# yupbank/tensorframes

Hardware: AMD Instinct MI355X
Metric: rows/sec map_blocks MatMul on 10M-row DF at 1/2/4/8 MI355X (higher is better)
Workload: dtype fp32; 1 GPU; model=map_blocks relu(matmul(x[?,512], W[512,512])) float32, global_batch=10000000, seq_len=512, parallelism=dp1, partitions=4, rows=10000000

## Files before the change

### csrc/runtime/executor.cpp

```cpp
#include "executor.h"

#include <optional>
#include "device_pool.h"


#include <ATen/hip/HIPContext.h>
#include <c10/hip/HIPCachingAllocator.h>
#include <c10/hip/HIPGuard.h>
#include <hip/hip_runtime.h>
#include <rocprofiler-sdk-roctx/roctx.h>

#include <algorithm>
#include <array>
#include <atomic>
#include <chrono>
#include <condition_variable>
#include <deque>
#include <thread>
#include <unistd.h>
#include <cstdlib>
#include <set>
#include <unordered_map>
#include <sstream>

// ... 1271 lines not shown
  p.arenas[di] = std::move(ar);
}

void Program::refresh_consts(Plan& p, int di, void* stream) {
  p.stale.erase(di);
  auto& m = p.dev_consts[di];
  if (m.empty()) return;
  auto drop = [&]() {
    m.clear();
    p.arenas.erase(di);
    p.cap_reset = true;
  };
  if (di < 0) {
    m.clear();
    return;
  }
  auto ait = p.arenas.find(di);
  if (ait == p.arenas.end()) return drop();
  Plan::Arena& ar = ait->second;
  std::set<int> in_arena;
  for (auto& it : ar.items) in_arena.insert(std::get<0>(it));
  for (auto& kv : m)
    if (!in_arena.count(kv.first) && kv.second.numel() > 0) return drop();
  at::Tensor host = at::empty({ar.dev.numel()}, at::TensorOptions().dtype(at::kByte).pinned_memory(true));
  auto* hp = static_cast<uint8_t*>(host.data_ptr());
  for (auto& it : ar.items) {
    const TensorRef& r = std::get<1>(it);
    const auto& v = p.infos[r.node][r.index].value;
    if (!v) return drop();
    at::Tensor c = v->contiguous();
    if (static_cast<size_t>(c.nbytes()) != std::get<3>(it)) return drop();
    std::memcpy(hp + std::get<2>(it), c.data_ptr(), c.nbytes());
  }
  hipStream_t s = static_cast<hipStream_t>(stream);
  for (void* us : p.used_streams[di])
    if (us && us != stream) (void)hipStreamSynchronize(static_cast<hipStream_t>(us));
  {
    c10::hip::HIPStreamGuard sg(c10::hip::getStreamFromExternal(s, static_cast<c10::DeviceIndex>(di)));
    ar.dev.copy_(host, true);
  }
  void*& ev = const_events_[{di, stream}];
  if (!ev) {
    hipEvent_t e;
    TFA_CHECK(hipEventCreateWithFlags(&e, hipEventDisableTiming) == hipSuccess, "hipEventCreate failed");
    ev = e;
  }
  (void)hipEventRecord(static_cast<hipEvent_t>(ev), s);
}

std::shared_ptr<Program> Program::rebind(const std::map<std::string, at::Tensor>& values) {
  static const bool timing = [] {
    const char* e = std::getenv("TFA_PLAN_TIMING");
    return e && std::string(e) == "3";
  }();
  const auto t0 = std::chrono::steady_clock::now();
  auto g = g_->with_values(values);
  const auto t1 = std::chrono::steady_clock::now();
  auto p = std::make_shared<Program>(std::move(g), fetch_names_, feed_names_);
  const auto t2 = std::chrono::steady_clock::now();
  p->adopt(*this);
  if (timing) {
    const auto t3 = std::chrono::steady_clock::now();
    auto us = [](auto a, auto b) { return std::chrono::duration<double, std::micro>(b - a).count(); };
    std::fprintf(stderr, "[tfa rebind] with_values %.1fus program %.1fus adopt %.1fus\n", us(t0, t1), us(t1, t2),
                 us(t2, t3));
  }
  return p;
}

bool Program::adopt(Program& old) {
  if (&old == this) return false;
  if (g_->structure_key() != old.g_->structure_key() || g_->nodes().size() != old.g_->nodes().size())
    return false;
  if (fetch_names_ != old.fetch_names_ || feed_names_ != old.feed_names_ || order_ != old.order_) return false;
  if (!host_op_error_.empty() || !old.host_op_error_.empty()) return false;
  std::scoped_lock lk(mu_, old.mu_, const_mu_, old.const_mu_);
  if (!plans_.empty()) return false;
  for (auto& kv : old.plans_) {
    if (!kv.second->synth_consts.empty()) return false;
    if (kv.second.use_count() != 1) return false;
  }
  std::vector<std::pair<std::shared_ptr<Plan>, Graph::Infos>> fresh;
  const std::vector<char>& prm = g_->parameter_consts();
  std::vector<char> redo(g_->nodes().size(), 0);
  for (int n : order_) {
    char t = prm[n];
    for (auto& r : g_->node(n).inputs) t = t || redo[r.node];
    redo[n] = t;
  }
  for (auto& kv : old.plans_) {
    Plan& p = *kv.second;
    Graph::Infos ni = p.infos.size() == g_->nodes().size() ? g_->infer_update(order_, p.infos, redo, true)
                                                           : g_->infer(order_, p.feed_infos, true);
    for (auto& cs : p.const_slots) {
      const TensorRef& r = cs.second;
      const TensorInfo& a = p.infos[r.node][r.index];
      const TensorInfo& b = ni[r.node][r.index];
      if (a.dtype != b.dtype || a.shape.dims != b.shape.dims || !b.value || !a.value ||
          a.value->sizes() != b.value->sizes())
        return false;
    }
    fresh.emplace_back(kv.second, std::move(ni));
  }
  for (auto& [pp, ni] : fresh) {
    Plan& p = *pp;
    for (auto& cs : p.const_slots) {
      const TensorRef& r = cs.second;
      p.infos[r.node][r.index].value = ni[r.node][r.index].value;
    }
    for (size_t n = 0; n < redo.size() && n < p.infos.size(); ++n)
      if (redo[n])
        for (size_t k = 0; k < p.infos[n].size() && k < ni[n].size(); ++k) p.infos[n][k].value = ni[n][k].value;
    for (auto& kv : p.dev_consts)
      if (!kv.second.empty()) p.stale.insert(kv.first);
  }
  plans_ = std::move(old.plans_);
  old.plans_.clear();
  old.graph_consts_.clear();
  for (auto& kv : old.const_events_) {
    void*& ev = const_events_[kv.first];
    if (ev) (void)hipEventDestroy(static_cast<hipEvent_t>(ev));
    ev = kv.second;
  }
  old.const_events_.clear();
  stats_.plans_adopted += static_cast<int64_t>(plans_.size());
  return true;
}

void Program::wait_consts(const at::Device& dev, void* stream) {
  std::lock_guard<std::mutex> lk(const_mu_);
  if (const_events_.empty()) return;
  const int di = dev.index();
  hipStream_t s = static_cast<hipStream_t>(stream);
  for (auto it = const_events_.begin(); it != const_events_.end();) {
    hipEvent_t e = static_cast<hipEvent_t>(it->second);
    if (it->first.first != di) {
      ++it;
      continue;
    }
    if (hipEventQuery(e) == hipSuccess) {
      (void)hipEventDestroy(e);
      it = const_events_.erase(it);
      continue;
    }
    if (it->first.second != stream && !dev_stream_capturing(s)) (void)hipStreamWaitEvent(s, e, 0);
    ++it;
  }
}

Program::~Program() {
  {
    std::lock_guard<std::mutex> lk(pipe_mu_);
    drop_pipe(false);
  }
  for (auto& kv : const_events_) (void)hipEventDestroy(static_cast<hipEvent_t>(kv.second));
}

std::vector<at::Tensor> Program::execute(Plan& p, const std::vector<at::Tensor>& inputs, void* stream) {
  const auto t_exec = std::chrono::steady_clock::now();
  auto epi_steps = [](const Step& st, const std::vector<at::Tensor>& slots) {
    std::vector<EpiStep> ep;
    for (const auto& e : st.epi) {
      EpiStep x;
      x.code = e.code;
      x.kind = e.kind;
      x.act = e.act;
      x.s = e.s;
      if (e.slot >= 0) x.t = slots[e.slot].contiguous();
      ep.push_back(std::move(x));
    }
    return ep;
  };
  const OpRegistry& reg = OpRegistry::get();
  at::Device dev = inputs.empty() ? at::Device(at::kCPU) : inputs[0].device();
  bool gpu = dev.is_cuda();
  for (auto& t : inputs)
    TFA_CHECK(t.device() == dev, "all inputs must live on the same device");
  std::vector<at::Tensor> slots(p.nslots);
  for (size_t i = 0; i < inputs.size(); ++i) slots[p.feed_slots[i]] = inputs[i].contiguous();
  if (!p.stale.empty()) {
    std::lock_guard<std::mutex> lk(const_mu_);
    const int di = gpu ? dev.index() : -1;
    if (p.stale.count(di)) refresh_consts(p, di, stream);
  }
  for (auto& cs : p.const_slots) slots[cs.first] = device_const(p, cs.first, dev, stream);
  if (gpu) {
    wait_consts(dev, stream);
    std::lock_guard<std::mutex> lk(const_mu_);
    p.last_stream[dev.index()] = stream;
    if (!dev_stream_capturing(static_cast<hipStream_t>(stream))) p.used_streams[dev.index()].insert(stream);
  }
  for (auto& sc : p.synth_consts) {
    std::lock_guard<std::mutex> lk(const_mu_);
    auto& m = p.dev_consts[dev.is_cuda() ? dev.index() : -1];
    auto it = m.find(sc.first);
    if (it == m.end()) it = m.emplace(sc.first, dev.is_cuda() ? sc.second.to(dev) : sc.second).first;
    slots[sc.first] = it->second;
  }
  const bool timing = gpu && g_step_timing.load(std::memory_order_relaxed) &&
                      !dev_stream_capturing(static_cast<hipStream_t>(stream));
  for (auto& st : p.steps) {
    const Node& nd = g_->node(st.node);
    ExecCtx c{nd, {}, {}, &st.out_info, &st.in_info, gpu, stream};
    for (int s : st.in_slots) c.in.push_back(slots[s]);
    c.out.resize(st.out_info.size());
    StepRec rec;
    if (timing) {
      TFA_CHECK(hipEventCreate(&rec.a) == hipSuccess, "hipEventCreate failed");
      TFA_CHECK(hipEventCreate(&rec.b) == hipSuccess, "hipEventCreate failed");
      TFA_CHECK(hipEventRecord(rec.a, static_cast<hipStream_t>(stream)) == hipSuccess, "hipEventRecord failed");
    }
    {
      std::unique_ptr<RangeGuard> rg;
      if (gpu) rg = std::make_unique<RangeGuard>(nd.op + ":" + nd.name);
      try {
        if (st.kind == Step::FUSED) {
          TFA_CHECK(gpu, "internal: fused step in a host plan");
          Plan::Fused& fe = *p.fused_regions[st.fused];
          const int di = dev.index();
          jit::Kernel kern;
          {
            std::lock_guard<std::mutex> lk(fe.mu);
            auto kit = fe.kernels.find(di);
            if (kit == fe.kernels.end()) {
              hipStreamCaptureStatus cs = hipStreamCaptureStatusNone;
              (void)hipStreamIsCapturing(static_cast<hipStream_t>(stream), &cs);
              TFA_CHECK(cs == hipStreamCaptureStatusNone, "fused kernel not loaded before graph capture");
              kit = fe.kernels.emplace(di, jit::get(fe.region.source, fe.region.entry)).first;
            }
            kern = kit->second;
          }
          std::vector<void*> outs;
          for (size_t k = 0; k < st.out_slots.size(); ++k) {
            c.out[k] = c.alloc_out(static_cast<int>(k));
            outs.push_back(c.out[k].data_ptr());
          }
          std::vector<const void*> ptrs;
          for (size_t k = 0; k < c.in.size(); ++k) {
            if (!c.in[k].is_contiguous()) c.in[k] = materialize(c, c.in[k]);
            ptrs.push_back(c.in[k].data_ptr());
          }
          std::vector<int64_t> w = fused_args(fe.region, ptrs, outs);
          TFA_CHECK(fe.region.grid >= 1 && fe.region.grid < (int64_t(1) << 31), "fused kernel: grid out of range");
          jit::launch(kern, static_cast<unsigned>(fe.region.grid), fe.region.block, w.data(),
                      w.size() * sizeof(int64_t), static_cast<hipStream_t>(stream));
        } else if (st.kind == Step::OP && gpu && !st.preplaced.empty()) {
          if (st.alias_slot >= 0) {
            at::Tensor& whole = slots[st.alias_slot];
            if (!whole.defined())
              whole = dev_empty(dims_or_throw(st.alias_info->shape, "concat output"), at::kFloat, dev,
                                static_cast<hipStream_t>(stream));
            slots[st.out_slots[0]] = whole.narrow(whole.dim() - 1, st.alias_offset, st.out_info[0].shape.dims.back());
          }
          at::Tensor& out = slots[st.out_slots[0]];
          TFA_CHECK(out.defined(), "internal: concat output not allocated by its producers");
          int64_t off = 0;
          const int64_t ax = out.dim() - 1;
          for (size_t v = 0; v < st.preplaced.size(); ++v) {
            const int64_t len = c.in[v].size(ax);
            if (!st.preplaced[v] && len > 0) gpu_copy(c.in[v], out.narrow(ax, off, len), stream_of(c));
            off += len;
          }
          c.out[0] = out;
        } else if (st.kind == Step::OP && gpu && (st.bias_slot >= 0 || st.act || st.alias_slot >= 0) &&
                   (nd.op == "AvgPool" || nd.op == "MaxPool")) {
          at::Tensor out;
          if (st.alias_slot >= 0) {
            at::Tensor& whole = slots[st.alias_slot];
            if (!whole.defined())
              whole = dev_empty(dims_or_throw(st.alias_info->shape, "concat output"), at::kFloat, dev,
                                static_cast<hipStream_t>(stream));
            out = whole.narrow(whole.dim() - 1, st.alias_offset, st.out_info[0].shape.dims.back());
          } else {
            out = c.alloc_out(0);
          }
          at::Tensor bias;
          if (st.bias_slot >= 0) bias = slots[st.bias_slot].contiguous();
          run_pool_fused(c, nd.op == "MaxPool", c.in[0], st.bias_slot >= 0 ? &bias : nullptr, st.act, out);
          c.out[0] = out;
        } else if (st.kind == Step::OP) {
          reg.find(nd.op)->compute(c);
        } else if (!st.sibs.empty()) {
          TFA_CHECK(gpu, "internal: sibling-fused conv in a host plan");
          std::vector<at::Tensor> outs;
          for (size_t k = 0; k < st.sibs.size(); ++k) {
            const Step::Sib& sb = st.sibs[k];
            if (sb.alias_slot >= 0) {
              at::Tensor& whole = slots[sb.alias_slot];
              if (!whole.defined())
                whole = dev_empty(dims_or_throw(sb.alias_info->shape, "concat output"), at::kFloat, dev,
                                  static_cast<hipStream_t>(stream));
              outs.push_back(whole.narrow(whole.dim() - 1, sb.alias_offset, sb.oc));
            } else {
              outs.push_back(c.alloc_out(static_cast<int>(k)));
            }
          }
          at::Tensor bias;
          if (st.bias_slot >= 0) bias = slots[st.bias_slot];
          std::vector<int> acts;
          for (const auto& sb : st.sibs) acts.push_back(sb.act);
          run_conv2d_siblings(c, c.in[0], c.in[1], st.bias_slot >= 0 ? &bias : nullptr, st.act, outs, acts,
                              st.wino_slot >= 0 ? &slots[st.wino_slot] : nullptr);
          for (size_t k = 0; k < outs.size(); ++k) c.out[k] = outs[k];
        } else if (gpu && st.alias_slot >= 0) {
          at::Tensor& whole = slots[st.alias_slot];
          if (!whole.defined())
// ... 544 lines not shown
    std::unique_lock<std::mutex> lk(mu);
    cv.wait(lk, [&] { return posted; });
    for (auto& j : jobs) {
      if (!j) continue;
      try {
        j->wait();
      } catch (const std::exception& e) {
        if (error.empty()) error = e.what();
      }
      j.reset();
    }
    TFA_CHECK(error.empty(), "packed output expansion failed: ", error);
  }

  std::mutex mu;
  std::condition_variable cv;
  bool posted = false;
  std::string error;
  std::vector<std::shared_ptr<unpack::Job>> jobs;
};

namespace {

class PackLander {
 public:
  static PackLander& get() {
    std::lock_guard<std::mutex> lk(inst_mu());
    if (!inst()) inst().reset(new PackLander());
    return *inst();
  }
  static void shutdown() {
    std::unique_ptr<PackLander> p;
    {
      std::lock_guard<std::mutex> lk(inst_mu());
      p = std::move(inst());
    }
    p.reset();
  }
  void submit(std::shared_ptr<PackLanding> l) {
    {
      std::lock_guard<std::mutex> lk(mu_);
      q_.push_back(std::move(l));
    }
    cv_.notify_one();
  }
  ~PackLander() {
    {
      std::lock_guard<std::mutex> lk(mu_);
      stop_ = true;
    }
    cv_.notify_all();
    thread_.join();
  }

 private:
  PackLander() : thread_([this] { loop(); }) {}
  static std::mutex& inst_mu() {
    static std::mutex m;
    return m;
  }
  static std::unique_ptr<PackLander>& inst() {
    static std::unique_ptr<PackLander> p;
    return p;
  }
  void loop() {
    for (;;) {
      std::shared_ptr<PackLanding> l;
      {
        std::unique_lock<std::mutex> lk(mu_);
        cv_.wait(lk, [&] { return stop_ || !q_.empty(); });
        if (q_.empty()) return;
        l = std::move(q_.front());
        q_.pop_front();
      }
      std::string err;
      std::vector<std::shared_ptr<unpack::Job>> jobs;
      const hipError_t e = hipEventSynchronize(l->ev);
      if (e != hipSuccess) {
        err = std::string("D2H of a packed chunk: ") + hipGetErrorString(e);
      } else {
        try {
          for (auto& t : l->tasks) jobs.push_back(unpack::global_pool().post_unpack(t.packed, t.out, t.rows, t.wpr));
        } catch (const std::exception& ex) {
          err = ex.what();
        }
      }
      {
        std::lock_guard<std::mutex> lk(l->mu);
        l->jobs = std::move(jobs);
        l->error = err;
        l->posted = true;
      }
      l->cv.notify_all();
    }
  }
  std::mutex mu_;
  std::condition_variable cv_;
  std::deque<std::shared_ptr<PackLanding>> q_;
  bool stop_ = false;
  std::thread thread_;
};

std::atomic<int>& pack_outputs_state() {
  static std::atomic<int> v([] {
    const char* e = std::getenv("TFA_PACK_OUTPUTS");
    if (!e) return 1;
    std::string s(e);
    for (auto& c : s) c = static_cast<char>(std::tolower(static_cast<unsigned char>(c)));
    return (s == "1" || s == "true" || s == "yes" || s == "on") ? 1 : 0;
  }());
  return v;
}

struct PipeHandle {
  hipEvent_t done = nullptr;
  std::vector<std::shared_ptr<PackLanding>> landings;
};

}

void set_pack_outputs(bool on) { pack_outputs_state().store(on ? 1 : 0); }
void set_pack_dense_fraction(double t) { g_pack_dense_fraction.store(t > 0 ? t : kPackDenseFraction); }
double pack_dense_fraction() { return g_pack_dense_fraction.load(); }
bool pack_outputs() { return pack_outputs_state().load() != 0; }

void shutdown_pack_runtime() {
  PackLander::shutdown();
  unpack::shutdown_pool();
}

void Program::drop_pipe(bool synced) {
  if (!pipe_) return;
  if (pipe_->device >= 0) {
    c10::hip::HIPGuard guard(static_cast<c10::DeviceIndex>(pipe_->device));
    if (!synced) {
      (void)hipStreamSynchronize(copy_stream(pipe_->device, 0));
      (void)hipStreamSynchronize(copy_stream(pipe_->device, 1));
      (void)hipDeviceSynchronize();
    }
    for (auto& l : pipe_->landing)
      if (l) {
        try {
          l->wait();
        } catch (const std::exception&) {
        }
      }
    for (hipEvent_t e : pipe_->ev_comp) (void)hipEventDestroy(e);
    for (hipEvent_t e : pipe_->ev_d2h) (void)hipEventDestroy(e);
    for (hipEvent_t e : pipe_->ev_land) (void)hipEventDestroy(e);
  }
  pipe_.reset();
}

void pipeline_wait(int64_t handle) {
  if (!handle) return;
  std::unique_ptr<PipeHandle> h(reinterpret_cast<PipeHandle*>(handle));
  const hipError_t e = hipEventSynchronize(h->done);
  (void)hipEventDestroy(h->done);
  std::string err;
  for (auto& l : h->landings) {
    try {
      l->wait();
    } catch (const std::exception& ex) {
      if (err.empty()) err = ex.what();
    }
  }
  HIP_OK(e);
  TFA_CHECK(err.empty(), err);
}

int64_t Program::run_chunked(const std::vector<std::vector<at::Tensor>>& seg_inputs,
                             const std::vector<std::vector<at::Tensor>>& seg_outputs,
                             int64_t chunk_rows, int device, int depth, bool wait) {
  TFA_CHECK(host_op_error_.empty(), host_op_error_);
  TFA_CHECK(seg_inputs.size() == seg_outputs.size(), "segments mismatch");
  TFA_CHECK(chunk_rows > 0, "chunk_rows must be > 0");
  depth = std::max(2, std::min(depth, 4));
  c10::hip::HIPGuard guard(static_cast<c10::DeviceIndex>(device));
  at::Device dev(at::kCUDA, static_cast<c10::DeviceIndex>(device));
  auto compute = c10::hip::getCurrentHIPStream(device);
  auto h2d = c10::hip::getStreamFromExternal(copy_stream(device, 0), static_cast<c10::DeviceIndex>(device));
  auto d2h = c10::hip::getStreamFromExternal(copy_stream(device, 1), static_cast<c10::DeviceIndex>(device));
  auto t0 = std::chrono::steady_clock::now();

  struct Chunk {
    size_t seg;
    int64_t start, rows;
  };
  std::vector<Chunk> chunks;
  for (size_t s = 0; s < seg_inputs.size(); ++s) {
    TFA_CHECK(seg_inputs[s].size() == feed_nodes_.size(), "segment ", s, ": expected ",
              feed_nodes_.size(), " inputs");
    TFA_CHECK(seg_outputs[s].size() == fetches_.size(), "segment ", s, ": expected ",
              fetches_.size(), " outputs");
    int64_t rows = seg_inputs[s].empty() ? 0 : seg_inputs[s][0].size(0);
    for (auto& t : seg_inputs[s]) {
      TFA_CHECK(t.size(0) == rows, "segment inputs disagree on rows");
      TFA_CHECK(!t.is_cuda() && t.is_contiguous(), "run_chunked inputs must be contiguous host tensors");
    }
    for (auto& t : seg_outputs[s])
      TFA_CHECK(!t.is_cuda() && t.is_contiguous() && t.size(0) == rows,
                "run_chunked outputs must be contiguous host tensors with ", rows, " rows");
    for (int64_t st = 0; st < rows; st += chunk_rows) chunks.push_back({s, st, std::min(chunk_rows, rows - st)});
  }
  if (chunks.empty()) return 0;
  std::lock_guard<std::mutex> plk(pipe_mu_);
  size_t nin = feed_nodes_.size();
  {
    std::vector<std::vector<int64_t>> shapes;
    std::vector<at::ScalarType> dts;
    for (size_t i = 0; i < nin; ++i) {
      auto sz = seg_inputs[chunks[0].seg][i].sizes().vec();
      sz.erase(sz.begin());
      shapes.push_back(sz);
      dts.push_back(seg_inputs[chunks[0].seg][i].scalar_type());
    }
    const bool fits = pipe_ && pipe_->device == device && pipe_->depth == depth && pipe_->shapes == shapes &&
                      pipe_->dtypes == dts && pipe_->rows >= chunk_rows;
    if (!fits) {
      drop_pipe(false);
      pipe_ = std::make_unique<Pipe>();
      pipe_->device = device;
      pipe_->depth = depth;
      pipe_->rows = chunk_rows;
      pipe_->shapes = shapes;
      pipe_->dtypes = dts;
      pipe_->ring.resize(depth);
      for (int d = 0; d < depth; ++d)
        for (size_t i = 0; i < nin; ++i) {
          std::vector<int64_t> sz = shapes[i];
          sz.insert(sz.begin(), chunk_rows);
          pipe_->ring[d].push_back(dev_empty(sz, dts[i], dev, compute.stream()));
        }
      order_copy_after_compute(h2d.stream(), compute.stream());
      pipe_->ev_comp.resize(depth);
      pipe_->ev_d2h.resize(depth);
      for (int d = 0; d < depth; ++d) {
        HIP_OK(hipEventCreateWithFlags(&pipe_->ev_comp[d], hipEventDisableTiming));
        HIP_OK(hipEventCreateWithFlags(&pipe_->ev_d2h[d], hipEventDisableTiming));
      }
      pipe_->used.assign(depth, false);
      pipe_->d2h_issued.assign(depth, true);
    }
  }
  Pipe& P = *pipe_;
  for (size_t s = 0; s < seg_inputs.size(); ++s)
    for (size_t i = 0; i < nin; ++i) {
      auto sz = seg_inputs[s][i].sizes().vec();
      sz.erase(sz.begin());
      TFA_CHECK(sz == P.shapes[i] && seg_inputs[s][i].scalar_type() == P.dtypes[i],
                "run_chunked: segments disagree on the row shape / dtype of feed ", i);
    }
  std::vector<hipEvent_t> ev_h2d(depth);
  for (int d = 0; d < depth; ++d) HIP_OK(hipEventCreateWithFlags(&ev_h2d[d], hipEventDisableTiming));
  int64_t h2d_bytes = 0, d2h_bytes = 0, d2h_dense_bytes = 0;
  const size_t nf = fetches_.size();
  if (pack_dense_.size() != nf) pack_dense_.assign(nf, 0);
  std::vector<char> packing(nf, 0), probe_only(nf, 0);
  std::vector<int64_t> fetch_wpr(nf, 0);
  if (pack_outputs()) {
    bool any = false;
    for (size_t j = 0; j < nf; ++j) {
      const at::Tensor& dst = seg_outputs[chunks[0].seg][j];
      const int64_t rb = dst.numel() / std::max<int64_t>(dst.size(0), 1) * dst.element_size();
      if (rb <= 0 || rb % 4 != 0) continue;
      fetch_wpr[j] = rb / 4;
      packing[j] = 1;
      probe_only[j] = pack_dense_[j];
      any = true;
    }
    if (any && P.packed.empty()) {
      P.packed.assign(depth, std::vector<at::Tensor>(nf));
      P.stage.assign(kPackStages, std::vector<at::Tensor>(nf));
      P.landing.assign(kPackStages, nullptr);
      P.ev_land.resize(kPackStages);
      for (auto& e : P.ev_land) HIP_OK(hipEventCreateWithFlags(&e, hipEventDisableTiming));
      P.counts = empty_pinned({static_cast<int64_t>(depth * nf)}, at::kLong);
    }
    for (size_t j = 0; j < nf; ++j) {
      if (!packing[j]) continue;
      const int64_t need = static_cast<int64_t>(pack_layout(P.rows, fetch_wpr[j]).max_bytes);
      if (!P.packed[0][j].defined()) {
        for (int d = 0; d < depth; ++d) P.packed[d][j] = dev_empty({need}, at::kByte, dev, compute.stream());
        for (int k = 0; k < kPackStages; ++k) P.stage[k][j] = empty_pinned({need}, at::kByte);
      } else if (P.packed[0][j].numel() < need) {
        packing[j] = 0;
      }
    }
  }
  const bool timed = stage_timers_enabled() && wait;
  std::vector<std::array<hipEvent_t, 6>> tev;
  auto stamp = [&](size_t ci, int k, hipStream_t s) {
    if (!timed) return;
    HIP_OK(hipEventCreate(&tev[ci][k]));
    HIP_OK(hipEventRecord(tev[ci][k], s));
  };
  if (timed) tev.assign(chunks.size(), std::array<hipEvent_t, 6>{});
  const int ncomp = (pipe_compute_streams() > 1 && chunks.size() > 1) ? 2 : 1;
  hipStream_t cstr[2] = {compute.stream(), ncomp > 1 ? copy_stream(device, 2) : compute.stream()};
  hipEvent_t fork_ev = nullptr;
  if (ncomp > 1) {
    HIP_OK(hipEventCreateWithFlags(&fork_ev, hipEventDisableTiming));
    HIP_OK(hipEventRecord(fork_ev, compute.stream()));
    HIP_OK(hipStreamWaitEvent(cstr[1], fork_ev, 0));
  }
  struct PendingD2H {
    bool active = false;
    size_t ci = 0;
    int slot = 0;
    std::vector<at::Tensor> outs;
    std::vector<char> packed;
    bool any_packed = false;
  };
  std::vector<std::shared_ptr<PackLanding>> call_landings;
  uint64_t* const counts = P.counts.defined() ? reinterpret_cast<uint64_t*>(P.counts.data_ptr()) : nullptr;
  auto issue_d2h = [&](PendingD2H& pd) {
    const Chunk& ch = chunks[pd.ci];
    const int slot = pd.slot;
    std::shared_ptr<PackLanding> landing;
    int stage = -1;
    if (pd.any_packed) {
      HIP_OK(hipEventSynchronize(P.ev_comp[slot]));
      stage = static_cast<int>(P.stage_next++ % kPackStages);
      if (P.landing[stage]) {
        std::shared_ptr<PackLanding> prev = std::move(P.landing[stage]);
        prev->wait();
      }
      landing = std::make_shared<PackLanding>();
      landing->ev = P.ev_land[stage];
    }
    HIP_OK(hipStreamWaitEvent(d2h.stream(), P.ev_comp[slot], 0));
    stamp(pd.ci, 4, d2h.stream());
    for (size_t j = 0; j < pd.outs.size(); ++j) {
      at::Tensor o = pd.outs[j];
      const at::Tensor& dst = seg_outputs[ch.seg][j];
      int64_t row_bytes = dst.numel() / std::max<int64_t>(dst.size(0), 1) * dst.element_size();
      char* dp = static_cast<char*>(dst.data_ptr()) + ch.start * row_bytes;
      d2h_dense_bytes += ch.rows * row_bytes;
      if (pd.packed[j]) {
        const PackLayout L = pack_layout(ch.rows, fetch_wpr[j]);
        const uint64_t total = counts[slot * nf + j];
        TFA_CHECK(total <= static_cast<uint64_t>(ch.rows * fetch_wpr[j]), "fetch '", fetch_names_[j],
                  "': packed ", total, " words of ", ch.rows * fetch_wpr[j]);
        const size_t bytes = L.values_off + static_cast<size_t>(total) * 4;
        HIP_OK(hipMemcpyAsync(P.stage[stage][j].data_ptr(), P.packed[slot][j].data_ptr(), bytes,
                              hipMemcpyDeviceToHost, d2h.stream()));
        d2h_bytes += static_cast<int64_t>(bytes);
        landing->tasks.push_back({P.stage[stage][j].data_ptr(), dp, ch.rows, fetch_wpr[j]});
        const bool dense =
            static_cast<double>(bytes) > g_pack_dense_fraction.load() * static_cast<double>(ch.rows * row_bytes);
        if (dense) {
          packing[j] = 0;
          pack_dense_[j] = 1;
        } else if (pack_dense_[j]) {
          pack_dense_[j] = 0;
          probe_only[j] = 0;
          packing[j] = 1;
        }
        continue;
      }
      if (!o.is_cuda()) o = o.to(dev);
      if (ch.rows * row_bytes)
        HIP_OK(hipMemcpyAsync(dp, o.data_ptr(), ch.rows * row_bytes, hipMemcpyDeviceToHost, d2h.stream()));
      dev_record_stream(o, d2h.stream());
      d2h_bytes += ch.rows * row_bytes;
    }
    stamp(pd.ci, 5, d2h.stream());
    HIP_OK(hipEventRecord(P.ev_d2h[slot], d2h.stream()));
    P.d2h_issued[slot] = true;
    if (landing) {
      HIP_OK(hipEventRecord(landing->ev, d2h.stream()));
      P.landing[stage] = landing;
      call_landings.push_back(landing);
      PackLander::get().submit(landing);
      stats_.chunks_packed++;
    }
    pd.outs.clear();
    pd.active = false;
  };
  PendingD2H lagged;
  for (size_t ci = 0; ci < chunks.size(); ++ci) {
    const hipStream_t cs = cstr[ci % ncomp];
    const Chunk& ch = chunks[ci];
    const int slot = static_cast<int>(P.next++ % depth);
    if (P.used[slot]) {
      TFA_CHECK(P.d2h_issued[slot], "run_chunked: slot ", slot, " reused before its D2H was issued");
      HIP_OK(hipStreamWaitEvent(h2d.stream(), P.ev_comp[slot], 0));
      HIP_OK(hipStreamWaitEvent(h2d.stream(), P.ev_d2h[slot], 0));
    }
    P.d2h_issued[slot] = false;
    std::vector<at::Tensor> dev_in;
    stamp(ci, 0, h2d.stream());
    for (size_t i = 0; i < nin; ++i) {
      const at::Tensor& src = seg_inputs[ch.seg][i];
      int64_t row_bytes = src.numel() / std::max<int64_t>(src.size(0), 1) * src.element_size();
      at::Tensor dst = P.ring[slot][i].narrow(0, 0, ch.rows);
      const char* sp = static_cast<const char*>(src.data_ptr()) + ch.start * row_bytes;
      if (ch.rows * row_bytes)
        HIP_OK(hipMemcpyAsync(dst.data_ptr(), sp, ch.rows * row_bytes, hipMemcpyHostToDevice, h2d.stream()));
      h2d_bytes += ch.rows * row_bytes;
      dev_in.push_back(dst);
    }
    stamp(ci, 1, h2d.stream());
    HIP_OK(hipEventRecord(ev_h2d[slot], h2d.stream()));
    HIP_OK(hipStreamWaitEvent(cs, ev_h2d[slot], 0));
    std::vector<at::Tensor> outs;
    stamp(ci, 2, cs);
    {
      RangeGuard rg("chunk_compute");
      auto p = plan_for(dev_in);
      outs = execute(*p, dev_in, cs);
    }
    stamp(ci, 3, cs);
    PendingD2H pd;
    pd.active = true;
    pd.ci = ci;
    pd.slot = slot;
    pd.packed.assign(nf, 0);
    for (size_t j = 0; j < outs.size(); ++j) {
      const at::Tensor& o = outs[j];
      const at::Tensor& dst = seg_outputs[ch.seg][j];
      int64_t row_bytes = dst.numel() / std::max<int64_t>(dst.size(0), 1) * dst.element_size();
      TFA_CHECK(o.size(0) == ch.rows && o.numel() * o.element_size() == ch.rows * row_bytes,
                "fetch '", fetch_names_[j], "' produced ", o.size(0), " rows for a chunk of ", ch.rows);
      if (!packing[j] || ch.rows == 0 || row_bytes != 4 * fetch_wpr[j]) continue;
      bool plain = o.is_cuda() && o.is_contiguous();
      for (size_t i = 0; plain && i < nin; ++i) {
        const char* r0 = static_cast<const char*>(P.ring[slot][i].data_ptr());
        const char* op = static_cast<const char*>(o.data_ptr());
        if (op >= r0 && op < r0 + P.ring[slot][i].numel() * P.ring[slot][i].element_size()) plain = false;
      }
      if (!plain) continue;
      if (!pd.any_packed && P.used[slot])
        HIP_OK(hipStreamWaitEvent(cs, P.ev_d2h[slot], 0));
      k::pack_words(o.data_ptr(), ch.rows, fetch_wpr[j], P.packed[slot][j].data_ptr(), cs);
      HIP_OK(hipMemcpyAsync(counts + slot * nf + j, P.packed[slot][j].data_ptr(), 8, hipMemcpyDeviceToHost, cs));
      pd.packed[j] = 1;
      pd.any_packed = true;
      if (probe_only[j]) packing[j] = 0;
    }
    pd.outs = std::move(outs);
    HIP_OK(hipEventRecord(P.ev_comp[slot], cs));
    P.used[slot] = true;
    stats_.chunks++;
    if (lagged.active) issue_d2h(lagged);
    if (pd.any_packed)
      lagged = std::move(pd);
    else
      issue_d2h(pd);
  }
  if (lagged.active) issue_d2h(lagged);
  if (ncomp > 1) {
    HIP_OK(hipEventRecord(fork_ev, cstr[1]));
    HIP_OK(hipStreamWaitEvent(compute.stream(), fork_ev, 0));
    HIP_OK(hipEventDestroy(fork_ev));
  }
  int64_t handle = 0;
  if (wait) {
    HIP_OK(hipStreamSynchronize(h2d.stream()));
    HIP_OK(hipStreamSynchronize(compute.stream()));
    HIP_OK(hipStreamSynchronize(d2h.stream()));
    std::string err;
    for (auto& l : call_landings) {
      try {
        l->wait();
      } catch (const std::exception& ex) {
        if (err.empty()) err = ex.what();
      }
    }
    drop_pipe(true);
    TFA_CHECK(err.empty(), err);
  } else {
    auto h = std::make_unique<PipeHandle>();
    HIP_OK(hipEventCreateWithFlags(&h->done, hipEventDisableTiming));
    HIP_OK(hipEventRecord(h->done, d2h.stream()));
    h->landings = std::move(call_landings);
    handle = reinterpret_cast<int64_t>(h.release());
  }
  for (int d = 0; d < depth; ++d) hipEventDestroy(ev_h2d[d]);
  double stage_ms[3] = {0, 0, 0};
  for (auto& e : tev) {
    for (int k = 0; k < 3; ++k) {
      float ms = 0.f;
      if (hipEventElapsedTime(&ms, e[2 * k], e[2 * k + 1]) == hipSuccess) stage_ms[k] += ms;
    }
    for (hipEvent_t ev : e) hipEventDestroy(ev);
  }
  auto t1 = std::chrono::steady_clock::now();
  stats_.runs++;
  stats_.h2d_bytes += h2d_bytes;
  stats_.d2h_bytes += d2h_bytes;
  stats_.d2h_dense_bytes += d2h_dense_bytes;
  stats_.wall_ms += std::chrono::duration<double, std::milli>(t1 - t0).count();
  stats_.h2d_ms += stage_ms[0];
  stats_.compute_ms += stage_ms[1];
  stats_.d2h_ms += stage_ms[2];
  return handle;
}

std::vector<at::Tensor> Program::run_chunked_reduce(const std::vector<std::vector<at::Tensor>>& seg_inputs,
                                                    int64_t chunk_rows, int device, int depth) {
  TFA_CHECK(host_op_error_.empty(), host_op_error_);
  TFA_CHECK(chunk_rows > 0, "chunk_rows must be > 0");
  depth = std::max(2, std::min(depth, 4));
  c10::hip::HIPGuard guard(static_cast<c10::DeviceIndex>(device));
  at::Device dev(at::kCUDA, static_cast<c10::DeviceIndex>(device));
  auto compute = c10::hip::getCurrentHIPStream(device);
  auto h2d = c10::hip::getStreamFromExternal(copy_stream(device, 0), static_cast<c10::DeviceIndex>(device));
  auto t0 = std::chrono::steady_clock::now();
  struct Chunk {
    size_t seg;
    int64_t start, rows;
  };
  std::vector<Chunk> chunks;
  for (size_t s = 0; s < seg_inputs.size(); ++s) {
    TFA_CHECK(seg_inputs[s].size() == feed_nodes_.size(), "segment ", s, ": expected ", feed_nodes_.size(), " inputs");
    const int64_t rows = seg_inputs[s].empty() ? 0 : seg_inputs[s][0].size(0);
    for (auto& t : seg_inputs[s]) {
      TFA_CHECK(t.size(0) == rows, "segment inputs disagree on rows");
      TFA_CHECK(!t.is_cuda() && t.is_contiguous(), "run_chunked_reduce inputs must be contiguous host tensors");
    }
    for (int64_t st = 0; st < rows; st += chunk_rows) chunks.push_back({s, st, std::min(chunk_rows, rows - st)});
  }
  TFA_CHECK(!chunks.empty(), "run_chunked_reduce: no rows");
  const size_t nin = feed_nodes_.size();
  std::vector<std::vector<at::Tensor>> ring(depth);
  for (int d = 0; d < depth; ++d)
    for (size_t i = 0; i < nin; ++i) {
      auto sz = seg_inputs[0][i].sizes().vec();
      sz[0] = chunk_rows;
      ring[d].push_back(dev_empty(sz, seg_inputs[0][i].scalar_type(), dev, compute.stream()));
    }
  order_copy_after_compute(h2d.stream(), compute.stream());
  std::vector<hipEvent_t> ev_h2d(depth), ev_comp(depth);
  for (int d = 0; d < depth; ++d) {
    HIP_OK(hipEventCreateWithFlags(&ev_h2d[d], hipEventDisableTiming));
    HIP_OK(hipEventCreateWithFlags(&ev_comp[d], hipEventDisableTiming));
  }
  std::vector<bool> used(depth, false);
  std::vector<at::Tensor> acc;
  int64_t h2d_bytes = 0;
  for (size_t ci = 0; ci < chunks.size(); ++ci) {
    const Chunk& ch = chunks[ci];
    const int slot = static_cast<int>(ci % depth);
    if (used[slot]) HIP_OK(hipStreamWaitEvent(h2d.stream(), ev_comp[slot], 0));
    std::vector<at::Tensor> dev_in;
    for (size_t i = 0; i < nin; ++i) {
      const at::Tensor& src = seg_inputs[ch.seg][i];
      const int64_t row_bytes = src.numel() / std::max<int64_t>(src.size(0), 1) * src.element_size();
      at::Tensor dst = ring[slot][i].narrow(0, 0, ch.rows);
      const char* sp = static_cast<const char*>(src.data_ptr()) + ch.start * row_bytes;
      if (ch.rows * row_bytes)
        HIP_OK(hipMemcpyAsync(dst.data_ptr(), sp, ch.rows * row_bytes, hipMemcpyHostToDevice, h2d.stream()));
      h2d_bytes += ch.rows * row_bytes;
      dev_in.push_back(dst);
    }
    HIP_OK(hipEventRecord(ev_h2d[slot], h2d.stream()));
    HIP_OK(hipStreamWaitEvent(compute.stream(), ev_h2d[slot], 0));
    std::vector<at::Tensor> outs;
    {
      RangeGuard rg("chunk_reduce");
      auto p = plan_for(dev_in);
      outs = execute(*p, dev_in, compute.stream());
    }
    if (acc.empty()) {
      for (auto& o : outs) {
        auto sz = o.sizes().vec();
        sz.insert(sz.begin(), static_cast<int64_t>(chunks.size()));
        acc.push_back(dev_empty(sz, o.scalar_type(), dev, compute.stream()));
      }
    }
    for (size_t j = 0; j < outs.size(); ++j) {
      at::Tensor o = outs[j].is_cuda() ? outs[j].contiguous() : outs[j].to(dev);
      at::Tensor dst = acc[j].select(0, static_cast<int64_t>(ci));
      TFA_CHECK(o.numel() == dst.numel(), "fetch '", fetch_names_[j], "' changed shape between chunks");
      const int64_t nb = o.numel() * o.element_size();
      if (nb) HIP_OK(hipMemcpyAsync(dst.data_ptr(), o.data_ptr(), nb, hipMemcpyDeviceToDevice, compute.stream()));
    }
    HIP_OK(hipEventRecord(ev_comp[slot], compute.stream()));
    used[slot] = true;
    stats_.chunks++;
  }
  HIP_OK(hipStreamSynchronize(h2d.stream()));
  for (int d = 0; d < depth; ++d) {
    hipEventDestroy(ev_h2d[d]);
    hipEventDestroy(ev_comp[d]);
  }
  auto t1 = std::chrono::steady_clock::now();
  stats_.runs++;
  stats_.h2d_bytes += h2d_bytes;
  stats_.wall_ms += std::chrono::duration<double, std::milli>(t1 - t0).count();
  return acc;
}

std::vector<std::string> Program::fused_sources(const std::vector<at::Tensor>& inputs) {
  auto p = build_plan(inputs, true);
  std::vector<std::string> out;
  for (auto& f : p->fused_regions) out.push_back(f->region.source);
  return out;
}

ExecStats Program::stats() const { return stats_; }
void Program::reset_stats() { stats_ = ExecStats(); }

std::string Program::describe_plan(const std::vector<at::Tensor>& inputs, bool as_gpu) {
  auto p = as_gpu ? build_plan(inputs, true) : plan_for(inputs);
  std::ostringstream os;
  os << "plan: " << p->steps.size() << " steps, " << p->const_slots.size() << " constants, "
     << p->fused << " fused epilogues, " << p->fused_regions.size() << " fused regions";
  if (p->fused_siblings) os << ", " << p->fused_siblings << " sibling convs fused";
  if (p->wino_convs) os << ", " << p->wino_convs << " Winograd filters";
  {
    const std::string why = graph_blocker(*p);
    os << (why.empty() ? ", graphable" : ", not graphable (" + why + ")");
  }
  os << "\n";
  for (auto& st : p->steps) {
    const Node& nd = g_->node(st.node);
    if (st.kind == Step::FUSED) {
      const FusedRegion& rg = p->fused_regions[st.fused]->region;
      os << "  FUSED" << (rg.kind == 1 ? "-ROWRED " : " ") << nd.name << " [" << rg.expr << "] "
         << rg.leaves.size() << " inputs " << rg.outputs.size() << " outputs " << st.out_info[0].shape.str();
      os << (rg.idx64 ? " idx64" : " idx32");
      if (rg.kind == 1) os << (rg.wave ? " wave" : " thread");
      os << " leaves[";
      static const char* leaf_kinds[] = {"contiguous", "scalar", "strided"};
      for (size_t k = 0; k < rg.leaves.size(); ++k) os << (k ? "," : "") << leaf_kinds[rg.leaves[k].kind];
      os << "]\n";
      continue;
    }
    os << "  " << (st.kind == Step::GEMM ? "GEMM" : st.kind == Step::CONV ? "CONV" : "OP  ") << ' '
       << nd.op << ' ' << nd.name;
    if (st.out_node != st.node) os << " -> " << g_->node(st.out_node).name;
    if (st.bias_slot >= 0) os << " +bias";
    if (st.act) os << " +" << act_name(st.act);
    if (!st.epi.empty()) {
      static const char* codes[] = {"add", "sub", "rsub", "mul", "div", "rdiv", "max", "min", "act", "neg", "square", "abs"};
      static const char* kinds[] = {"", "scalar", "scalar", "col", "row", "full"};
      os << " +epi[";
// ... 146 lines not shown
```

### csrc/runtime/executor.h

```cpp
#pragma once

#include <ATen/ATen.h>
#include <hip/hip_runtime.h>

#include <map>
#include <tuple>
#include <memory>
#include <mutex>
#include <optional>
#include <string>
#include <vector>

#include "../ir/graph.h"

namespace tfa {

struct MonoidInfo {
  std::string fetch;
  std::string placeholder;
  std::string op;
};

struct ExecStats {
  int64_t runs = 0;
  int64_t kernels = 0;
  int64_t plans_built = 0;
  int64_t plans_adopted = 0;
  int64_t h2d_bytes = 0;
  int64_t d2h_bytes = 0;
  int64_t d2h_dense_bytes = 0;
  int64_t chunks = 0;
  int64_t chunks_packed = 0;
  double h2d_ms = 0, compute_ms = 0, d2h_ms = 0, wall_ms = 0;
  double plan_ms = 0;
  double exec_ms = 0;
  int64_t graphs_captured = 0, graph_replays = 0, graph_failures = 0, graphs_declined = 0;
  int64_t graph_busy = 0;
};

struct PackLanding;

class Program {
 public:
  Program(std::shared_ptr<Graph> g, const std::vector<std::string>& fetches,
          const std::vector<std::string>& feeds);
  ~Program();

  const std::vector<std::string>& fetch_names() const { return fetch_names_; }
  const std::vector<std::string>& feed_names() const { return feed_names_; }

  Graph::Infos analyze(const std::map<std::string, TensorInfo>& feed_infos) const;
  bool row_separable(const std::map<std::string, TensorInfo>& feed_infos) const;
  std::vector<MonoidInfo> monoids() const;

  bool adopt(Program& old);
  std::shared_ptr<Program> rebind(const std::map<std::string, at::Tensor>& values);

  std::vector<at::Tensor> run(const std::vector<at::Tensor>& inputs);

  std::vector<std::vector<at::Tensor>> run_concurrent(const std::vector<std::vector<at::Tensor>>& inputs_list,
                                                      int max_streams = 4);

  int64_t run_chunked(const std::vector<std::vector<at::Tensor>>& seg_inputs,
                      const std::vector<std::vector<at::Tensor>>& seg_outputs, int64_t chunk_rows,
                      int device, int depth, bool wait = true);

  void release_pipeline() {
    std::lock_guard<std::mutex> lk(pipe_mu_);
    drop_pipe(false);
  }

  std::vector<at::Tensor> run_chunked_reduce(const std::vector<std::vector<at::Tensor>>& seg_inputs,
                                             int64_t chunk_rows, int device, int depth);

  ExecStats stats() const;
  void reset_stats();
  std::string describe_plan(const std::vector<at::Tensor>& inputs, bool as_gpu = false);
  std::vector<std::string> fused_sources(const std::vector<at::Tensor>& inputs);

 private:
  std::string host_op_error_;
  struct Step;
  struct Plan;
 public:
  struct AliasUseSink {
    virtual ~AliasUseSink() = default;
    virtual void record_use(hipStream_t s) = 0;
  };

 private:
  std::shared_ptr<Plan> plan_for(const std::vector<at::Tensor>& inputs);
  std::shared_ptr<Plan> build_plan(const std::vector<at::Tensor>& inputs, bool force_gpu);
  std::vector<at::Tensor> execute(Plan& p, const std::vector<at::Tensor>& inputs, void* stream);
  at::Tensor device_const(Plan& p, int slot, const at::Device& dev, void* stream);
  void upload_consts(Plan& p, std::map<int, at::Tensor>& m, const at::Device& dev, void* stream);
  void wait_consts(const at::Device& dev, void* stream);
  void refresh_consts(Plan& p, int di, void* stream);
  bool graphable(const Plan& p) const;
  std::string graph_blocker(const Plan& p) const;
  std::vector<at::Tensor> run_graph(Plan& p, const std::vector<at::Tensor>& inputs);
  std::optional<std::vector<at::Tensor>> run_ptr_graph(Plan& p, const std::vector<at::Tensor>& inputs,
                                                       int64_t bytes);

  std::shared_ptr<Graph> g_;
  std::vector<std::string> fetch_names_, feed_names_;
  std::vector<TensorRef> fetches_;
  std::vector<int> feed_nodes_;
  std::vector<int> order_;
  std::mutex mu_;
  static constexpr size_t kMaxPlans = 256;
  std::map<std::string, std::shared_ptr<Plan>> plans_;
  std::mutex const_mu_;
  std::map<std::tuple<int, int, int>, at::Tensor> graph_consts_;
  std::map<std::pair<int, void*>, void*> const_events_;
  ExecStats stats_;
  struct Pipe {
    int device = -1, depth = 0;
    int64_t rows = 0;
    std::vector<std::vector<int64_t>> shapes;
    std::vector<at::ScalarType> dtypes;
    std::vector<std::vector<at::Tensor>> ring;
    std::vector<hipEvent_t> ev_comp, ev_d2h;
    std::vector<bool> used;
    int64_t next = 0;
    std::vector<bool> d2h_issued;
    std::vector<std::vector<at::Tensor>> packed;
    at::Tensor counts;
    std::vector<std::vector<at::Tensor>> stage;
    std::vector<hipEvent_t> ev_land;
    std::vector<std::shared_ptr<PackLanding>> landing;
    int64_t stage_next = 0;
  };
  std::mutex pipe_mu_;
  std::unique_ptr<Pipe> pipe_;
  std::vector<char> pack_dense_;
  void drop_pipe(bool synced);
};

struct StepTiming {
  std::string node, op, label;
  double flops, bytes;
  float ms;
};
void set_step_timing(bool on);
bool step_timing();
std::vector<StepTiming> read_step_timing();

void pipeline_wait(int64_t handle);
void set_pack_outputs(bool on);
bool pack_outputs();
void set_pack_dense_fraction(double t);
double pack_dense_fraction();
void shutdown_pack_runtime();

at::Tensor empty_pinned(const std::vector<int64_t>& sizes, at::ScalarType dt);
void trim_pinned_pool();
size_t pinned_pool_cached_bytes();
std::vector<size_t> pinned_pool_stats();
void pin_host_tensor(const at::Tensor& t);
void unpin_host_tensor(const at::Tensor& t);
hipStream_t copy_stream(int device, int which);
void set_debug_sync(bool on);
bool get_debug_sync();

}
```

Before: 26.17 million rows/s.

## Issue H2D copies ahead of compute and reuse stage timer events

Host-to-device copies for upcoming chunks are now enqueued up to depth-2 chunks ahead of the compute loop. The copy stream can then stay busy while earlier chunks compute, instead of each chunk's upload being issued only when its own compute is issued. Stage timing events are pooled and reused across calls rather than created and destroyed per chunk, and H2D stage time is measured from a derived start event. A guard drops the pipe if the loop fails partway. The run-ahead adds slot-reuse ordering complexity and assumes depth is at least 2.

```diff
diff --git a/csrc/runtime/executor.cpp b/csrc/runtime/executor.cpp
--- a/csrc/runtime/executor.cpp
+++ b/csrc/runtime/executor.cpp
@@ -1447,6 +1447,7 @@
   {
     std::lock_guard<std::mutex> lk(pipe_mu_);
     drop_pipe(false);
+    drop_timers();
   }
   for (auto& kv : const_events_) (void)hipEventDestroy(static_cast<hipEvent_t>(kv.second));
 }
@@ -2297,6 +2298,13 @@
   pipe_.reset();
 }
 
+void Program::drop_timers() {
+  if (timer_events_.empty()) return;
+  c10::hip::HIPGuard guard(static_cast<c10::DeviceIndex>(timer_device_));
+  for (hipEvent_t e : timer_events_) (void)hipEventDestroy(e);
+  timer_events_.clear();
+}
+
 void pipeline_wait(int64_t handle) {
   if (!handle) return;
   std::unique_ptr<PipeHandle> h(reinterpret_cast<PipeHandle*>(handle));
@@ -2435,9 +2443,19 @@
   }
   const bool timed = stage_timers_enabled() && wait;
   std::vector<std::array<hipEvent_t, 6>> tev;
+  size_t timer_next = 0;
+  if (timed && timer_device_ != device) {
+    drop_timers();
+    timer_device_ = device;
+  }
   auto stamp = [&](size_t ci, int k, hipStream_t s) {
     if (!timed) return;
-    HIP_OK(hipEventCreate(&tev[ci][k]));
+    if (timer_next == timer_events_.size()) {
+      hipEvent_t e;
+      HIP_OK(hipEventCreate(&e));
+      timer_events_.push_back(e);
+    }
+    tev[ci][k] = timer_events_[timer_next++];
     HIP_OK(hipEventRecord(tev[ci][k], s));
   };
   if (timed) tev.assign(chunks.size(), std::array<hipEvent_t, 6>{});
@@ -2524,9 +2542,15 @@
     pd.active = false;
   };
   PendingD2H lagged;
-  for (size_t ci = 0; ci < chunks.size(); ++ci) {
-    const hipStream_t cs = cstr[ci % ncomp];
-    const Chunk& ch = chunks[ci];
+  struct Staged {
+    int slot = 0;
+    std::vector<at::Tensor> dev_in;
+  };
+  std::vector<Staged> staged(chunks.size());
+  size_t h2d_front = 0;
+  const size_t run_ahead = static_cast<size_t>(depth - 2);
+  auto enqueue_h2d = [&](size_t hi) {
+    const Chunk& ch = chunks[hi];
     const int slot = static_cast<int>(P.next++ % depth);
     if (P.used[slot]) {
       TFA_CHECK(P.d2h_issued[slot], "run_chunked: slot ", slot, " reused before its D2H was issued");
@@ -2534,8 +2558,8 @@
       HIP_OK(hipStreamWaitEvent(h2d.stream(), P.ev_d2h[slot], 0));
     }
     P.d2h_issued[slot] = false;
-    std::vector<at::Tensor> dev_in;
-    stamp(ci, 0, h2d.stream());
+    staged[hi].slot = slot;
+    if (hi < static_cast<size_t>(depth)) stamp(hi, 0, h2d.stream());
     for (size_t i = 0; i < nin; ++i) {
       const at::Tensor& src = seg_inputs[ch.seg][i];
       int64_t row_bytes = src.numel() / std::max<int64_t>(src.size(0), 1) * src.element_size();
@@ -2544,10 +2568,24 @@
       if (ch.rows * row_bytes)
         HIP_OK(hipMemcpyAsync(dst.data_ptr(), sp, ch.rows * row_bytes, hipMemcpyHostToDevice, h2d.stream()));
       h2d_bytes += ch.rows * row_bytes;
-      dev_in.push_back(dst);
-    }
-    stamp(ci, 1, h2d.stream());
+      staged[hi].dev_in.push_back(dst);
+    }
+    stamp(hi, 1, h2d.stream());
     HIP_OK(hipEventRecord(ev_h2d[slot], h2d.stream()));
+  };
+  struct DrainOnFailure {
+    Program* prog;
+    bool armed = true;
+    ~DrainOnFailure() {
+      if (armed) prog->drop_pipe(false);
+    }
+  } drain_on_failure{this};
+  for (size_t ci = 0; ci < chunks.size(); ++ci) {
+    const hipStream_t cs = cstr[ci % ncomp];
+    const Chunk& ch = chunks[ci];
+    while (h2d_front < chunks.size() && h2d_front <= ci + run_ahead) enqueue_h2d(h2d_front++);
+    const int slot = staged[ci].slot;
+    const std::vector<at::Tensor> dev_in = std::move(staged[ci].dev_in);
     HIP_OK(hipStreamWaitEvent(cs, ev_h2d[slot], 0));
     std::vector<at::Tensor> outs;
     stamp(ci, 2, cs);
@@ -2622,14 +2660,24 @@
     h->landings = std::move(call_landings);
     handle = reinterpret_cast<int64_t>(h.release());
   }
+  drain_on_failure.armed = false;
   for (int d = 0; d < depth; ++d) hipEventDestroy(ev_h2d[d]);
   double stage_ms[3] = {0, 0, 0};
-  for (auto& e : tev) {
+  auto later = [](hipEvent_t a, hipEvent_t b) {
+    float ms = 0.f;
+    return hipEventElapsedTime(&ms, a, b) == hipSuccess && ms > 0.f ? b : a;
+  };
+  auto h2d_start = [&](size_t ci) {
+    if (tev[ci][0]) return tev[ci][0];
+    return later(later(tev[ci - 1][1], tev[ci - depth][3]), tev[ci - depth][5]);
+  };
+  for (size_t ci = 0; ci < tev.size(); ++ci) {
+    const auto& e = tev[ci];
+    const hipEvent_t from[3] = {h2d_start(ci), e[2], e[4]};
     for (int k = 0; k < 3; ++k) {
       float ms = 0.f;
-      if (hipEventElapsedTime(&ms, e[2 * k], e[2 * k + 1]) == hipSuccess) stage_ms[k] += ms;
-    }
-    for (hipEvent_t ev : e) hipEventDestroy(ev);
+      if (hipEventElapsedTime(&ms, from[k], e[2 * k + 1]) == hipSuccess) stage_ms[k] += ms;
+    }
   }
   auto t1 = std::chrono::steady_clock::now();
   stats_.runs++;
diff --git a/csrc/runtime/executor.h b/csrc/runtime/executor.h
--- a/csrc/runtime/executor.h
+++ b/csrc/runtime/executor.h
@@ -68,6 +68,7 @@
   void release_pipeline() {
     std::lock_guard<std::mutex> lk(pipe_mu_);
     drop_pipe(false);
+    drop_timers();
   }
 
   std::vector<at::Tensor> run_chunked_reduce(const std::vector<std::vector<at::Tensor>>& seg_inputs,
@@ -135,6 +136,9 @@
   std::unique_ptr<Pipe> pipe_;
   std::vector<char> pack_dense_;
   void drop_pipe(bool synced);
+  std::vector<hipEvent_t> timer_events_;
+  int timer_device_ = -1;
+  void drop_timers();
 };
 
 struct StepTiming {
```

Result: no change. 25.99 million rows/s (-0.7%).
